# ddkang/avrecode

Hardware: AMD Instinct MI355X
Metric: input H.264 MB/s (compress+roundtrip) at 1/2/4/8 GPUs; bit-exact pass (higher is better)
Workload: dtype u8; 1 GPU; synthetic batch of independent 1080p CABAC I-slices (BASELINE configs[2]); slices_per_gpu=1024, model=parallel (the reference model reset per slice, SURVEY.md 7), input_bytes_per_gpu=261361164, recoded_bytes_C=258817967, bins=2511192484

## Files before the change

avrecode_amd/csrc/avr_walker.h:

```cpp
#pragma once
#include <type_traits>

#include "avr_slice_lds.h"

#define AVR_MB_LIKELY(x) (MODE == MODE_DECOMPRESS ? AVR_LIKELY(x) : (x))
#define AVR_MB_UNLIKELY(x) (MODE == MODE_DECOMPRESS ? AVR_UNLIKELY(x) : (x))

namespace avr {


template <int MODE, bool RM, bool FLD = false, bool P32 = false, bool SPL = false, bool SRD = false>
struct Walker {
  static constexpr bool DEC = MODE == MODE_COMPRESS || MODE == MODE_TRACE;
  const HotTables* T;
  const EngineTables* G;
  const avr_slice_desc* d;
  Shared* sh;
  typedef typename std::conditional<FLD, EdgeRec, EdgeCore>::type ERec;
  ERec* ring;
  uint32_t* mring;
  bool mring_global;
  uint16_t* est_g;
  uint8_t* frames;
  int64_t cur_off, prev_off;
  bool gmode;
  uint32_t* gsink;
  uint32_t gcount;
  InStream in;
  OutStream out;
  CabacDecoder cd;
  CabacEncoder ce;
  RecodedEncoder re;
  static constexpr bool VD = MODE == MODE_DECOMPRESS && !P32 && !RM && !SRD;
  typename std::conditional<P32, PDecoder, typename std::conditional<VD, VDecoder, RecodedDecoder>::type>::type rd;
  uint64_t rng;
  int W, H, mb_x, mb_y, slice_type, is_b, cat_, t8mode;
  int fld, fld_pic, my, ystep;
  int top_pending;
  AVR_FI int mrow() const { return FLD ? my : mb_y; }
  int mbaff;
  uint32_t pst, ring_cols;
  int left_ok, top_ok, last_dqp_nz;
  uint32_t cf, lf, tf;
  static constexpr uint32_t CF_8X8 = 0x80;
  uint32_t edge_src;
  int err, finished;
  uint32_t bins;
  int target_mbs, mbs_done, last_mb;
  int nref0, nref1, d8x8inf, x264_build, first_mb;
  const SeamRec* seam;
  uint8_t* snap;
  uint32_t* snap_count;
  uint32_t snap_cap, snap_n, snap_last, snap_q, split_bits, rec_stride, piece_mbs;
  int cut;
  AVR_FI bool seam_place(uint32_t bitpos, uint32_t offset, uint32_t* ce) const {
    if (bitpos < 26) return false;
    const uint32_t m = (bitpos - 10) >> 3, sb = m > 12 ? m - 12 : 0, e = (bitpos + 7) >> 3, r = 8 * e - bitpos;
    const uint32_t sub = offset << r;
    uint32_t borrow = 0, low = 0, q = ~0u, cache = 0;
    for (uint32_t j = e; j-- > sb;) {
      const uint32_t t = e - 1 - j;
      const uint32_t sbyte = t < 4 ? (sub >> (8 * t)) & 0xff : 0u;
      const uint32_t f = j < in.limit ? (uint32_t)in.g[j] : 0u;
      const uint32_t v = f - sbyte - borrow;
      borrow = v >> 31;
      const uint32_t z = v & 0xff;
      if (j >= m) low |= z << (8 * t);
      else if (q == ~0u && z != 0xff) q = j, cache = z;
    }
    if (borrow || q == ~0u) return false;
    const uint32_t lowbits = bitpos - 8 * m;
    ce[0] = (low >> r) & ((1u << lowbits) - 1);
    ce[1] = cd.range;
    ce[2] = m - 1 - q;
    ce[3] = cache;
    ce[4] = lowbits - 18;
    ce[5] = q;
    return true;
  }
  AVR_FI void seam_cut(int addr) {
    const uint32_t pos = cd_bitpos(cd);
    if (pos - snap_last < split_bits || (uint64_t)pos + split_bits / 2 > 8ull * d->payload_size) return;
    snap_last = pos;
    if (snap_n >= snap_cap) return;
    uint32_t ce[6];
    if (!seam_place(pos, cd.low >> cd.k, ce) || (snap_n && ce[5] <= snap_q)) return;
    snap_q = ce[5];
    rc_writeback();
    mc_store();
    uint32_t* r32 = (uint32_t*)(snap + (size_t)snap_n * rec_stride);
    const uint32_t lane = __lane_id();
    if (lane < 16) {
      const uint32_t v = lane == 0 ? (uint32_t)addr : lane == 1 ? (uint32_t)last_dqp_nz : lane == 2 ? cd.low
                       : lane == 3 ? cd.range : lane == 4 ? (uint32_t)cd.k : lane == 5 ? cd.next
                       : lane == 6 ? ce[0] : lane == 7 ? ce[1] : lane == 8 ? ce[2] : lane == 9 ? ce[3]
                       : lane == 10 ? ce[4] : lane == 11 ? ce[5] : 0u;
      r32[lane] = v;
    }
    const uint32_t* st = (const uint32_t*)sh->state;
    for (uint32_t i = lane; i < 256; i += 64) r32[16 + i] = st[i];
    const uint32_t* e = (const uint32_t*)ring;
    for (uint32_t i = lane; i < (uint32_t)W * 10; i += 64) r32[16 + 256 + i] = i % 10 ? e[i] : e[i] & ~kEdgeMringNz;
    snap_n++;
    if constexpr (MODE == MODE_COMPRESS) {
      push(OP_FINISH | OP_RESTART);
      publish();
      while (ld_volatile(&sh->fifo_tail[0]) != ring0.head) {
        __builtin_amdgcn_s_sleep(1);
      }
      for (uint32_t i = lane; i < (uint32_t)W * kMringDwords; i += 64) mring[i] = 0;
      wave_sync();
    }
  }
  uint32_t prio_cell, prio_cur;
  AVR_FI void update_prio() {
    const uint32_t pos = MODE == MODE_DECOMPRESS ? rd.next : cd.next;
    const uint32_t size = d->payload_size;
    const uint32_t rem = pos < size ? size - pos : 0u;
    cu_post(prio_cell, rem);
    const uint32_t p = cu_rank_prio(prio_cell, rem);
    if (p != prio_cur) {
      prio_cur = p;
      set_prio(p);
      if (__lane_id() == 0) *(volatile __attribute__((address_space(3))) uint32_t*)&sh->prio = p;
    }
  }
  RingOutT<MODE == MODE_DECOMPRESS> ring0;
  static constexpr bool kStageLevels = true;
// ... 418 lines not shown
        int sy, ry;
        left_src(fld, afrm, bottom, y4, 16, &sy, &ry);
        t8rows |= (((sy ? lb : lt) & F_T8) ? 1u : 0u) << y4;
      }
      int s = 0, dw = 0;
      if (L >= 1 && L < 13) {
        const int p = ((int)L - 1) >> 2;
        int r;
        left_src(fld, afrm, bottom, ((int)L - 1) & 3, (cat_ == 1 && p) ? 8 : 16, &s, &r);
        dw = 1 + p * 4 + min(r, 3);
      } else if (L >= 13 && L < 29) {
        const int k = ((int)L - 13) & 7;
        int r;
        left_src(fld, afrm, bottom, k >> 1, 16, &s, &r);
        dw = 13 + (((int)L - 13) >> 3) * 8 + r * 2 + (k & 1);
      } else if (L == 29 || L == 30 || L == 31) {
        s = s0;
        dw = (int)L;
      } else if (L >= 32 && L < 45) {
        s = bottom;
        dw = (int)L;
      }
      uint32_t v = L < 45 ? ((const uint32_t*)&lp[s])[dw] : 0u;
      const uint32_t v2 = (L >= 29 && L < 32) ? ((const uint32_t*)&lp[s2])[L] : 0u;
      if (L == 0) {
        v = t8rows | cbp << 16;
      } else if (L >= 13 && L < 29) {
        if (fld != (uint32_t)(!afrm)) v = scale_mvd(v, fld);
      } else if (L == 29 || L == 30 || L == 31) {
        const uint32_t b1 = (v >> (8 * ((r0 >> 1) * 2 + 1))) & 0xff, b3 = (v2 >> (8 * ((r2 >> 1) * 2 + 1))) & 0xff;
        v = (L == 31 ? 0u : 0xff00ffu) | b1 << 8 | b3 << 24;
        if (L != 31 && fld != (uint32_t)(!afrm)) v = scale_ref(v, fld);
      }
      if (L < 45) ((uint32_t*)&sh->left)[L] = v;
    }
    const int above = (at & F_DEC) != 0;
    const int sel = !fld ? (bottom ? 1 : above ? 2 : 0) : above ? ((!bottom && (at & F_FLD)) ? 1 : 2) : 0;
    const int msel = bottom ? 1 : above ? 2 : 0;
    uint32_t v = 0;
    if (L < 10 && sel) v = ((const uint32_t*)&pair_edge(sel - 1)[mb_x])[L];
    else if (L >= 10 && L < 23 && msel) v = ((const uint32_t*)&pair_edge(msel - 1)[mb_x])[L];
    const uint32_t t0 = __builtin_amdgcn_readlane(v, 0);
    if (sel && ((t0 & F_FLD) ? 1u : 0u) != fld) {
      if (L >= 4 && L < 8) v = scale_mvd(v, fld);
      else if (L == 8) v = scale_ref(v, fld);
    }
    if (L < 23) ((uint32_t*)&ring[mb_x])[L] = v;
    tf = t0;
    top_ok = sel != 0;
    wave_sync();
  }
  AVR_FI void mbaff_layer_begin() {
    const int bottom = (pst & PST_BOT) != 0;
    uint32_t fld = pst & PST_FLD;
    if (!bottom) {
      fld = mbaff_field_flag(fld);
      pst = (pst & ~PST_FLD) | fld;
    }
    if (fld) cf |= F_FLD;
    mbaff_view(bottom, fld);
  }

  AVR_FI int mnnz_left(int idx) const {
    if (RM) return frames[cur_off + ((int64_t)mrow() * W + mb_x - 1) * 52 + idx];
    return left_ok ? sh->left.mnnz[idx] : 0;
  }
  AVR_FI int mnnz_top(int idx) const {
    if (RM) return (FLD && top_pending) ? 0 : frames[cur_off + ((int64_t)(mrow() - 1) * W + mb_x) * 52 + idx];
    if (FLD && fld_pic) return 0;
    if constexpr (FLD) {
      return (top_ok | mbaff) ? ring[mb_x].mnnz[idx] : 0;
    } else {
      if (!top_ok) return 0;
      const uint32_t at = (uint32_t)mb_x * (kMringDwords * 4) + mring_dword((uint32_t)idx >> 2) * 4 + ((uint32_t)idx & 3);
      if (mring_global) return (tf & kEdgeMringNz) ? ((const __attribute__((address_space(1))) uint8_t*)mring)[at] : 0;
      return ((const __attribute__((address_space(3))) uint8_t*)mring)[at];
    }
  }
  AVR_FI int mnnz_prev(int idx) const {
    if (RM) return prev_off < 0 ? 0 : frames[prev_off + ((int64_t)mrow() * W + mb_x) * 52 + idx];
    return 0;
  }

  AVR_FI int nz_bits(int cat, int n, int max, int is_dc, int c422, int count) {
    const int bits = max > 16 ? 6 : max > 4 ? 4 : 2;
    if (MODE == MODE_COMPRESS && RM && gmode && !gsink) {
      gcount += (uint32_t)bits;
      return count & ((1 << bits) - 1);
    }
    int has_left, has_above, lv = 0, av = 0;
    if (n >= 48) {
      has_left = mb_x > 0;
      has_above = mrow() > 0;
      if (has_left) lv = mnnz_left(n);
      if (has_above) av = mnnz_top(n);
    } else {
      uint8_t L = T->nb_left[n], U = T->nb_up[n];
      int li = L & 63, ui = U & 63;
      if (max >= 32) { li &= ~3; ui &= ~3; }
      has_left = !(L & 128) || mb_x > 0;
      has_above = !(U & 128) || mrow() > 0;
      if (has_left) lv = (L & 128) ? mnnz_left(li) : sh->cur.mnnz[li];
      if (has_above) av = (U & 128) ? mnnz_top(ui) : sh->cur.mnnz[ui];
    }
    const int pv = mnnz_prev(n);
    const int t = (((cf & CF_8X8) || max > 32) ? 1 : 0) + 2 * is_dc + c422 + 4 * cat;
    if (MODE == MODE_COMPRESS) {
      const int i = (int)__lane_id();
      const int cur_bit = 1 << (i & 7);
      const int so_far = count & (cur_bit - 1);
      const int lb = has_left ? (lv >= cur_bit) : 2;
      const int ab = av ? (av >= cur_bit) : 2;
      const int pb = pv >= cur_bit;
      const int idx = kSigEst + (((((cur_bit - 1 + so_far) * 2 + pb) * 3 + lb) * 3 + ab) * 57 + t);
      push_v(op_model((count >> (i & 7)) & 1, OPM_CACHE, idx), (uint32_t)bits);
      return count & ((1 << bits) - 1);
    }
    if (MODE == MODE_DECOMPRESS) {
      const uint32_t L = __lane_id();
      const int i = 31 - __clz((int)L + 1);
      const int cur_bit = 1 << i;
      const int lb = has_left ? (lv >= cur_bit) : 2;
      const int ab = av ? (av >= cur_bit) : 2;
      const int pb = pv >= cur_bit;
      const uint32_t idx_v = kSigEst + ((((L * 2 + pb) * 3 + lb) * 3 + ab) * 57 + t);
      uint32_t e_v = 0, slot_v = 0;
      const bool hit = est_probe4(sh, idx_v, &e_v, &slot_v);
      const uint64_t hit_m = __ballot(hit);
      int so_far = 0;
      for (int k = 0; k < bits; k++) {
        const uint32_t j = (1u << k) - 1 + (uint32_t)so_far;
        const uint32_t idx = __builtin_amdgcn_readlane(idx_v, j);
        uint32_t e, slot;
        if ((hit_m >> j) & 1) {
          e = __builtin_amdgcn_readlane(e_v, j);
          slot = __builtin_amdgcn_readlane(slot_v, j);
        } else {
          e = est_load(sh, est_g, idx, &slot);
        }
        const int b = rdec(e);
        est_store(sh, est_g, idx, slot, est_update(e, b, 0x60));
        so_far |= b << k;
      }
      return so_far;
    }
    int so_far = 0;
    for (int i = 0; i < bits; i++) {
      const int cur_bit = 1 << i;
      const int lb = has_left ? (lv >= cur_bit) : 2;
      const int ab = av ? (av >= cur_bit) : 2;
      const int pb = pv >= cur_bit;
      const int idx = kSigEst + (((((cur_bit - 1 + so_far) * 2 + pb) * 3 + lb) * 3 + ab) * 57 + t);
      int b;
      if (MODE == MODE_COMPRESS) {
        b = (count >> i) & 1;
        push(op_model(b, OPM_CACHE, idx));
      } else {
        uint32_t slot;
        const uint32_t e = est_load(sh, est_g, idx, &slot);
        b = rdec(e);
        est_store(sh, est_g, idx, slot, est_update(e, b, 0x60));
      }
      if (b) so_far |= cur_bit;
    }
    return so_far;
  }

  AVR_FI int sig_est_index(int cat, int max, int is_dc, int c422, int zz, int nnz_m, int obs) const {
    if (max == 64) return T->sig_est_base[cat] + (T->sig8x8[zz] * 64 + nnz_m) * 64 + obs;
    int zo = (is_dc && c422) ? (zz < 2 ? 0 : zz < 4 ? 1 : 2) : zz;
    return T->sig_est_base[cat] + (zo * 16 + nnz_m) * 16 + obs;
  }

  AVR_FI int sig_map(int cat, int n, int max, int is_dc, int c422) {
    const int numc8x8 = cat_ == 2 ? 2 : 1;
    const int sb = T->sig_base[cat], lb = T->last_base[cat], seb = (int)opaque_u32((uint32_t)T->sig_est_base[cat]);
    const int bits = max > 16 ? 6 : max > 4 ? 4 : 2;
    const int mask = (1 << bits) - 1;
    int cnt = 0;
    if (DEC) {
      uint64_t sigmask = 0;
      int pos, end = max - 2;
      PROF_BEGIN(t3);
      if (MODE == MODE_TRACE) trace_map_begin(cat, n, max, is_dc, c422);
      auto map_loop = [&](auto K) {
        constexpr int k = decltype(K)::value;
        for (pos = 0; pos < max - 1; pos++) {
          int sc, lc;
          if constexpr (k == 2) {
            sc = (int)__builtin_amdgcn_readlane(sig8_v, (uint32_t)pos);
            lc = (int)__builtin_amdgcn_readlane(last8_v, (uint32_t)pos);
          } else if constexpr (k == 1) {
            sc = lc = min(pos / numc8x8, 2);
          } else {
            sc = lc = pos;
          }
          if (rdecide(sc)) {
            sigmask |= 1ull << pos;
            cnt++;
            if (rdecide(16 + lc)) { end = pos; break; }
          }
        }
      };
      if (max == 64) map_loop(std::integral_constant<int, 2>());
      else if (cat == 3) map_loop(std::integral_constant<int, 1>());
      else map_loop(std::integral_constant<int, 0>());
      if (pos == max - 1) cnt++;
      if (MODE == MODE_TRACE) trace_map_end();
      PROF_END(3, t3);
      if (MODE == MODE_COMPRESS) {
        PROF_BEGIN(t4);
        nz_bits(cat, n, max, is_dc, c422, cnt);
        PROF_END(4, t4);
        PROF_BEGIN(t5);
        const int nnz_m = cnt & mask;
        const int zz = (int)__lane_id();
        const int b = (int)((sigmask >> zz) & 1);
        const int obs = (int)__builtin_amdgcn_mbcnt_hi((uint32_t)(sigmask >> 32), __builtin_amdgcn_mbcnt_lo((uint32_t)sigmask, 0u));
        const int idx = sig_est_index(cat, max, is_dc, c422, zz, nnz_m, obs);
        push_v(op_model(b, OPM_CACHE | OPM_THR50, idx), (uint32_t)end + 1);
        PROF_END(5, t5);
      }
    } else if (MODE == MODE_DECOMPRESS) {
      PROF_BEGIN(t4);
      const int nnz_m = nz_bits(cat, n, max, is_dc, c422, 0);
      PROF_END(4, t4);
      PROF_BEGIN(t3);
      int pos;
      const uint32_t sop = opaque_u32((uint32_t)sb << 3 | OPK_DECISION << 1 | 1u << OPC_SHIFT_D);
      const uint32_t lop = opaque_u32((uint32_t)lb << 3 | OPK_DECISION << 1 | 2u << OPC_SHIFT_D);
      auto map_loop = [&](auto K) {
        constexpr int k = decltype(K)::value;
        constexpr int stride = k == 2 ? 64 : 16;
        uint32_t mk = 0;
        constexpr bool defer = k == 0;
        uint32_t dslot_v = 0, de_v = 0;
        for (pos = 0; pos < max - 1; pos++) {
          int sc, lc, zo;
          if constexpr (k == 2) {
            const uint32_t v = __builtin_amdgcn_readlane(sig8_v, (uint32_t)pos);
            sc = FLD ? (int)(v & 0xff) : (int)v;
            zo = FLD ? (int)(v >> 8) : (int)v;
            lc = (int)__builtin_amdgcn_readlane(last8_v, (uint32_t)pos);
          } else if constexpr (k == 1) {
            sc = lc = min(pos / numc8x8, 2);
            zo = (is_dc && c422) ? (pos < 2 ? 0 : pos < 4 ? 1 : 2) : pos;
          } else {
            sc = lc = zo = pos;
          }
          const int idx = seb + (zo * stride + nnz_m) * stride + cnt;
          uint32_t slot;
          uint32_t e = est_load(sh, est_g, idx, &slot, defer);
          int b = rdec(e);
          const uint32_t ne = est_update(e, b, 0x50);
          if (defer && AVR_LIKELY(slot >> 31)) {
            dslot_v = wlane(dslot_v, (uint32_t)pos, slot);
            de_v = wlane(de_v, (uint32_t)pos, ne);
          } else {
            est_store(sh, est_g, idx, slot, ne);
          }
          bins++;
          if constexpr (FLD) push(sop + ((uint32_t)sc << 3) + (uint32_t)b);
          else mk |= (uint32_t)b << (pos & 15);
          if (b) {
            cnt++;
            int last = nnz_m == cnt;
            bins++;
            if constexpr (FLD) push(lop + ((uint32_t)lc << 3) + (uint32_t)last);
            if (last) break;
          }
          if constexpr (!FLD && k == 2) {
            if ((pos & 15) == 15) {
              push(op_map(cat, 16, 0, mk));
              mk = 0;
            }
          }
        }
        if constexpr (defer) {
          if (dslot_v >> 31) sh->etab[dslot_v & 0xffff] = (dslot_v & 0xffff0000u) | de_v;
          wave_sync();
        }
        if constexpr (!FLD) {
          const int ended = pos < max - 1;
          push(op_map(cat, (pos & 15) + ended, ended, mk));
        }
      };
      if (max == 64) map_loop(std::integral_constant<int, 2>());
      else if (cat == 3) map_loop(std::integral_constant<int, 1>());
      else map_loop(std::integral_constant<int, 0>());
      if (pos == max - 1) cnt++;
      PROF_END(3, t3);
    } else {
      int pos;
      for (pos = 0; pos < max - 1; pos++) {
        int sc, lc;
        if (max == 64) {
          sc = (int)__builtin_amdgcn_readlane(sig8_v, (uint32_t)pos);
          lc = (int)__builtin_amdgcn_readlane(last8_v, (uint32_t)pos);
        }
        else if (cat == 3) { sc = lc = min(pos / numc8x8, 2); }
        else sc = lc = pos;
        if (rbin(sc, sb + sc)) {
          cnt++;
          if (rbin(16 + lc, lb + lc)) break;
        }
      }
      if (pos == max - 1) cnt++;
    }
    return cnt;
  }

  AVR_FI void residual_block(int cat, int n, int max, int is_dc, int c422, int p, int pw, int x4, int y4) {
    if (AVR_MB_UNLIKELY(err)) return;
    MbRec& cur = sh->cur;
    int coded = 1;
    if (max != 64 || cat_ == 3) {
      int nza, nzb;
      if (is_dc) {
        int bit = cat == 3 ? (0x40 << (n - 49)) : (0x100 << (n - 48));
        nza = (nb_cbp_left() & bit) != 0;
        nzb = (nb_cbp_top() & bit) != 0;
      } else {
        nza = nnz_left(p, pw, x4, y4) > 0;
        nzb = nnz_top(p, x4, y4) > 0;
      }
      rc_select(cat);
      coded = rbin(42 + nza + 2 * nzb, T->cbf_base[cat] + nza + 2 * nzb);
    }
    int cnt = 0;
    if (coded) {
      rc_select(cat);
      cnt = sig_map(cat, n, max, is_dc, c422);
      const int ab = (int)opaque_u32((uint32_t)T->abs_base[cat]);
      int gt1 = 0, eq1 = 0;
      PROF_BEGIN(t6);
      if constexpr (MODE == MODE_DECOMPRESS && !FLD) {
        for (int i = cnt - 1; i >= 0 && !err; i--) {
          int absl;
          const int i0 = gt1 ? 0 : min(4, 1 + eq1);
          if (!rdec_lane(32 + i0)) {
            absl = 1;
          } else {
            const int i1 = 5 + min(4 - (cat == 3), gt1);
            absl = 2;
            while (absl < 15 && rdec_lane(32 + i1)) absl++;
          }
          if (absl < 15) {
            push(op_level(cat, absl, rdec_bypass()));
          } else {
            push(op_level(cat, 15, 0));
            int k = 0;
            while (bypass(SE_LEVEL_SUFFIX, k)) {
              if (++k > 30) { err = AVR_SLICE_BAD_LEVEL; break; }
            }
            while (k-- > 0) bypass(SE_LEVEL_SUFFIX, 100);
            bypass(SE_OTHER, 0);
          }
          if (absl == 1) eq1++;
          else gt1++;
        }
      } else if constexpr (MODE == MODE_COMPRESS && kStageLevels) {
        const bool st = !(RM && gmode);
        auto lpush = [&](uint32_t op) {
          if (st) ring0.stage(op);
          else push(op);
        };
        auto lbyp = [&]() {
          bins++;
          const int b = cd_bypass(cd, in);
          lpush(op_model(b, 0, 1024));
          return b;
        };
        for (int i = cnt - 1; i >= 0 && !err; i--) {
          int absl;
          const int i0 = gt1 ? 0 : min(4, 1 + eq1);
          int b = rdecide(32 + i0);
          lpush(op_model(b, 0, ab + i0));
          if (!b) {
            absl = 1;
          } else {
            const int i1 = 5 + min(4 - (cat == 3), gt1);
            absl = 2;
            while (absl < 15) {
              b = rdecide(32 + i1);
              lpush(op_model(b, 0, ab + i1));
              if (!b) break;
              absl++;
            }
            if (absl >= 15) {
              int k = 0;
              while (lbyp()) {
                if (++k > 30) { err = AVR_SLICE_BAD_LEVEL; break; }
              }
              while (k-- > 0) lbyp();
            }
          }
          lbyp();
          if (absl == 1) eq1++;
          else gt1++;
        }
        if (st) ring0.flush_stage();
      } else
      for (int i = cnt - 1; i >= 0 && !err; i--) {
        int absl;
        const int i0 = gt1 ? 0 : min(4, 1 + eq1);
        if (!rbin(32 + i0, ab + i0)) {
          absl = 1;
        } else {
          const int i1 = 5 + min(4 - (cat == 3), gt1);
          absl = 2;
          while (absl < 15 && rbin(32 + i1, ab + i1)) absl++;
          if (absl >= 15) {
            int k = 0;
            while (bypass(SE_LEVEL_SUFFIX, k)) {
              if (++k > 30) { err = AVR_SLICE_BAD_LEVEL; break; }
            }
            int v = 1;
            while (k-- > 0) v += v + bypass(SE_LEVEL_SUFFIX, 100);
            absl = 14 + v;
          }
        }
        bypass(SE_OTHER, 0);
        if (absl == 1) eq1++;
        else gt1++;
      }
      PROF_END(6, t6);
      cur.mnnz[n] = (uint8_t)cnt;
      if (max > 32) cf |= CF_8X8;
    }
    if (is_dc) {
      if (cnt) cf |= (uint32_t)(cat == 3 ? (0x40 << (n - 49)) : (0x100 << (n - 48))) << 16;
    } else if (max == 64) {
      cur.nnz[p][y4 * 4 + x4] = cur.nnz[p][y4 * 4 + x4 + 1] = (uint8_t)cnt;
      cur.nnz[p][y4 * 4 + 4 + x4] = cur.nnz[p][y4 * 4 + 4 + x4 + 1] = (uint8_t)cnt;
    } else {
      cur.nnz[p][y4 * 4 + x4] = (uint8_t)cnt;
    }
  }

  AVR_FI void blk_pos(int n, int* x4, int* y4) const {
    int s = c_scan8[n];
    int row = s >> 3;
    *x4 = (s & 7) - 4;
    *y4 = row <= 4 ? row - 1 : row <= 9 ? row - 6 : row - 11;
  }

  AVR_FI int push_block(int nb, int cat, int n, int max, int is_dc, int c422, int p, int pw, int x4, int y4) {
    sh->blk[nb] = (uint32_t)cat | (uint32_t)n << 4 | (uint32_t)max << 10 | (uint32_t)is_dc << 17 |
                  (uint32_t)c422 << 18 | (uint32_t)p << 19 | (uint32_t)pw << 21 | (uint32_t)x4 << 24 |
                  (uint32_t)y4 << 26;
    return nb + 1;
  }
  AVR_FI int list_luma(int nb, int p, int i16, int cbp) {
    const int cat_dc = p == 0 ? 0 : p == 1 ? 6 : 10;
    const int cat_ac = cat_dc + 1, cat_4 = cat_dc + 2, cat_8 = p == 0 ? 5 : p == 1 ? 9 : 13;
    int x4, y4;
    if (i16) {
      nb = push_block(nb, cat_dc, 48 + p, 16, 1, 0, p, 4, 0, 0);
      if (cbp & 15)
        for (int i = 0; i < 16; i++) {
          blk_pos(16 * p + i, &x4, &y4);
          nb = push_block(nb, cat_ac, 16 * p + i, 15, 0, 0, p, 4, x4, y4);
        }
      return nb;
    }
    for (int i8 = 0; i8 < 4; i8++) {
      if (!(cbp & (1 << i8))) continue;
      if (cf & F_T8) {
        blk_pos(16 * p + 4 * i8, &x4, &y4);
        nb = push_block(nb, cat_8, 16 * p + 4 * i8, 64, 0, 0, p, 4, x4, y4);
      } else {
        for (int i4 = 0; i4 < 4; i4++) {
          int n = 16 * p + 4 * i8 + i4;
          blk_pos(n, &x4, &y4);
          nb = push_block(nb, cat_4, n, 16, 0, 0, p, 4, x4, y4);
        }
      }
    }
    return nb;
  }

  AVR_FI void residual(int i16, int cbp) {
    int nb = list_luma(0, 0, i16, cbp);
    if (cat_ == 3) {
      nb = list_luma(nb, 1, i16, cbp);
      nb = list_luma(nb, 2, i16, cbp);
    } else if (cat_ == 1 || cat_ == 2) {
      const int c422 = cat_ == 2;
      if (cbp & 0x30)
        for (int c = 0; c < 2; c++) nb = push_block(nb, 3, 49 + c, c422 ? 8 : 4, 1, c422, 1 + c, 2, 0, 0);
      if (cbp & 0x20)
        for (int c = 0; c < 2; c++)
          for (int i8 = 0; i8 < (c422 ? 2 : 1); i8++)
            for (int i = 0; i < 4; i++) {
              int n = 16 + 16 * c + 8 * i8 + i, x4, y4;
              blk_pos(n, &x4, &y4);
              nb = push_block(nb, 4, n, 15, 0, 0, 1 + c, 2, x4, y4);
            }
    }
    PROF_BEGIN(t2);
    for (int j = 0; j < nb && AVR_MB_LIKELY(!err); j++) {
      const uint32_t b = sh->blk[j];
      residual_block(b & 15, (b >> 4) & 63, (b >> 10) & 127, (b >> 17) & 1, (b >> 18) & 1, (b >> 19) & 3,
                     (b >> 21) & 7, (b >> 24) & 3, (b >> 26) & 3);
    }
    PROF_END(2, t2);
  }

  AVR_FI int ref_gt0(int list, int x4, int y4, int use_left) const {
    uint8_t dir;
    int r;
    if (use_left) {
      if (x4 > 0) {
        int b8 = (y4 >> 1) * 2 + ((x4 - 1) >> 1);
        dir = sh->cur.direct8[b8]; r = sh->cur.ref[list][b8];
      } else {
        if (!left_ok) return 0;
        int b8 = (y4 >> 1) * 2 + 1;
        dir = sh->left.direct8[b8]; r = sh->left.ref[list][b8];
      }
    } else {
      if (y4 > 0) {
        int b8 = ((y4 - 1) >> 1) * 2 + (x4 >> 1);
        dir = sh->cur.direct8[b8]; r = sh->cur.ref[list][b8];
      } else {
        if (!top_ok) return 0;
        dir = ring[mb_x].direct8[x4 >> 1]; r = ring[mb_x].ref[list][x4 >> 1];
      }
    }
    if (is_b && dir) return 0;
    return r > 0;
  }
  AVR_FI int decode_ref(int list, int x4, int y4) {
    int ctx = ref_gt0(list, x4, y4, 1) + 2 * ref_gt0(list, x4, y4, 0);
    int ref = 0;
    avr_limit = (list ? nref1 : nref0) - 1;
    while (bin(SE_REF, ref, 54 + ctx)) {
      ref++;
      ctx = (ctx >> 2) + 4;
      if (ref >= 32) { err = AVR_SLICE_BAD_REF_IDX; return 0; }
    }
    return ref;
  }
  AVR_FI int mvd_nb(int list, int comp, int x4, int y4, int use_left) const {
    if (use_left) {
      if (x4 > 0) return sh->cur.mvd[list][y4 * 4 + x4 - 1][comp];
      return left_ok ? sh->left.mvd[list][y4 * 4 + 3][comp] : 0;
    }
    if (y4 > 0) return sh->cur.mvd[list][(y4 - 1) * 4 + x4][comp];
    return top_ok ? ring[mb_x].mvd[list][x4][comp] : 0;
  }
  AVR_FI int decode_mvd(int list, int comp, int x4, int y4) {
    const int base = comp ? 47 : 40;
    const int amvd = mvd_nb(list, comp, x4, y4, 1) + mvd_nb(list, comp, x4, y4, 0);
    const int inc = amvd < 3 ? 0 : amvd <= 32 ? 1 : 2;
    if constexpr (MODE == MODE_DECOMPRESS && !FLD) {
      if (!rdec_mc(base + inc)) {
        push(op_mvd(comp, inc, 0, 0));
        return 0;
      }
      int mvd = 1, ctx = base + 3;
      while (mvd < 9 && rdec_mc(ctx)) {
        if (mvd < 4) ctx++;
        mvd++;
      }
// ... 333 lines not shown
  const int cols = (FLD && d->structure == AVR_STRUCT_MBAFF && (int)w.ring_cols >= 3 * w.W + 7) ? 3 * w.W + 7 : w.W;
  if (seam) {
    const uint32_t* e32 = (const uint32_t*)(seam + 1);
    for (int i = lane; i < w.W * kEdgeBytes / 4; i += nt) ring32[i] = i % 10 ? e32[i] : e32[i] & ~kEdgeMringNz;
    if (!w.mring_global)
      for (int i = lane; i < w.W * kMringDwords; i += nt) w.mring[i] = 0;
  } else {
    for (int i = lane; i < cols * (int)sizeof(typename Walker<MODE, RM, FLD, P32, SPL, SRD>::ERec) / 4; i += nt) ring32[i] = 0;
  }
  if (lane < 2) {
    w.sh->fifo_head[lane] = 0;
    w.sh->fifo_tail[lane] = 0;
  }
  __syncthreads();
}

template <int MODE, bool RM, bool FLD, bool P32, bool SPL, bool SRD>
AVR_FI void walk_slice(Walker<MODE, RM, FLD, P32, SPL, SRD>& w) {
  const avr_slice_desc* d = w.d;
  w.W = d->mb_width;
  w.H = (FLD && w.fld_pic) ? d->mb_height >> 1 : d->mb_height;
  w.slice_type = d->slice_type;
  w.is_b = d->slice_type == 1;
  w.cat_ = d->chroma_array_type;
  w.t8mode = d->transform_8x8_mode;
  w.nref0 = d->num_ref_idx_l0;
  w.nref1 = d->num_ref_idx_l1;
  w.d8x8inf = d->direct_8x8_inference;
  w.x264_build = d->x264_build;
  w.first_mb = d->first_mb;
  w.last_dqp_nz = 0;
  if constexpr (SPL) {
    if (w.seam) w.last_dqp_nz = (int)w.seam->last_dqp_nz;
  }
  w.err = 0;
  w.finished = 0;
  w.bins = 0;
  w.mbs_done = 0;
  int addr = d->first_mb;
  const int lane = threadIdx.x;
  const int npic = w.W * w.H;
  w.mb_x = addr % w.W;
  w.mb_y = addr / w.W;
  w.ystep = (FLD && w.fld_pic) ? 2 : 1;
  w.my = w.mb_y * w.ystep + (d->structure == AVR_STRUCT_BOTTOM_FIELD ? 1 : 0);
  w.mbaff = FLD && d->structure == AVR_STRUCT_MBAFF;
  w.pst = 0;
  if ((FLD && w.mbaff)) {
    if ((int)w.ring_cols < 3 * w.W + 7 || (addr & 1)) { w.err = AVR_SLICE_MBAFF_RING; return; }
    w.mb_x = (addr >> 1) % w.W;
    w.mb_y = (addr >> 1) / w.W;
    w.ystep = 2;
    w.my = 2 * w.mb_y;
  }
  {
    const int j = lane, ph_c = (w.cat_ == 2 || w.cat_ == 3) ? 4 : 2;
    int src = 0;
    if (j >= 1 && j < 4) src = 1 + (j - 1) * 4 + (j == 1 ? 3 : ph_c - 1);
    else if (j >= 4 && j < 8) src = 13 + ((j - 4) >> 1) * 8 + 6 + ((j - 4) & 1);
    else if (j == 8) src = 29;
    else if (j == 9) src = 31;
    else if (j >= 10 && j < 23) src = 32 + (j - 10);
    w.edge_src = (uint32_t)src;
  }
  for (;;) {
    if (AVR_MB_UNLIKELY(addr >= npic)) { w.err = AVR_SLICE_BAD_MB_ADDR; break; }
    if constexpr (SPL && MODE == MODE_COMPRESS) {
      if (AVR_MB_UNLIKELY(w.snap && w.mb_x == 0 && w.mbs_done > 0)) w.seam_cut(addr);
    }
    PROF_BEGINW(ps0);
    if (!(FLD && w.mbaff)) {
      w.left_ok = w.mb_x > 0 && addr - 1 >= w.first_mb;
      w.tf = *(const uint32_t*)&w.ring[w.mb_x];
      w.top_ok = (w.tf & F_DEC) != 0;
    } else if (!(w.pst & Walker<MODE, RM, FLD, P32, SPL, SRD>::PST_BOT)) {
      w.mbaff_pair_start();
    }
    w.cf = 0;
    {
      uint32_t* c32 = (uint32_t*)&w.sh->cur;
      if (lane < (int)sizeof(MbRec) / 4) c32[lane] = (lane == 29 || lane == 30) ? 0xffffffffu : 0u;
      wave_sync();
    }
    SPROF_ENDW(0, ps0);
#ifdef AVR_PROFILE
    w.sprofb[0]++;
#endif
    PROF_BEGINW(t1);
    w.decode_mb();
    PROF_ENDW(1, t1);
    PROF_BEGINW(t7);
    if (AVR_MB_UNLIKELY(w.err)) break;
    w.cf |= F_DEC;
    w.mbs_done++;
    w.last_mb = addr + 1 >= npic;
    wave_sync();
    {
      const uint32_t* c32 = (const uint32_t*)&w.sh->cur;
      const uint32_t v = c32[lane < 45 ? lane : 44];
      const uint32_t ve = c32[w.edge_src], ref1 = c32[30];
      const uint32_t ev = lane == 8 ? (ve >> 16) | (ref1 & 0xffff0000u) : lane == 9 ? ve >> 16 : ve;
      if (!(FLD && w.mbaff)) {
        uint32_t* l32 = (uint32_t*)&w.sh->left;
        if (lane < 45) l32[lane] = v;
        uint32_t* e32 = (uint32_t*)&w.ring[w.mb_x];
        if constexpr (FLD) {
          if (lane < 23) e32[lane] = lane == 0 ? (w.cf & 0xffff017fu) : ev;
        } else {
          const bool mz = !RM && w.mring_global &&
                          __ballot(lane >= 10 && lane < 23 && ((kMringUsed >> (lane - 10)) & 1) && ev != 0) != 0;
          if (lane < 10) e32[lane] = lane == 0 ? ((w.cf & 0xffff017fu) | (mz ? kEdgeMringNz : 0u)) : ev;
          else if (!RM && lane < 23 && ((kMringUsed >> (lane - 10)) & 1)) {
            const uint32_t at = (uint32_t)w.mb_x * kMringDwords + mring_dword((uint32_t)lane - 10);
            if (w.mring_global) {
              if (mz) ((__attribute__((address_space(1))) uint32_t*)w.mring)[at] = ev;
            } else {
              ((__attribute__((address_space(3))) uint32_t*)w.mring)[at] = ev;
            }
          }
        }
        w.lf = w.cf;
      } else {
        const int bot = (w.pst & Walker<MODE, RM, FLD, P32, SPL, SRD>::PST_BOT) != 0;
        uint32_t* e32 = (uint32_t*)&w.pair_edge(bot)[w.mb_x];
        if (lane < 23) e32[lane] = lane == 0 ? (w.cf & 0xffff017fu) : ev;
        uint32_t* pr = (uint32_t*)w.pair_rec();
        const uint32_t t = pr[lane < 45 ? lane : 44];
        if (!bot) {
          if (lane < 45) pr[lane] = lane == 0 ? w.cf : v;
        } else if (lane < 45) {
          pr[45 + lane] = t;
          pr[90 + lane] = lane == 0 ? w.cf : v;
        }
      }
      if (RM) {
        uint32_t* f32 = (uint32_t*)(w.frames + w.cur_off + ((int64_t)w.mrow() * w.W + w.mb_x) * 52);
        if (lane >= 32 && lane < 45) f32[lane - 32] = v;
      }
      wave_sync();
    }
    PROF_ENDW(7, t7);
    PROF_BEGINW(ps7);
    if (MODE == MODE_COMPRESS || MODE == MODE_DECOMPRESS) {
      w.publish();
      if (!RM) w.update_prio();
    }
    const int eos = (!(FLD && w.mbaff) || (w.pst & Walker<MODE, RM, FLD, P32, SPL, SRD>::PST_BOT)) ? w.terminate(SE_EOS) : 0;
    SPROF_ENDW(7, ps7);
    if (AVR_MB_UNLIKELY(eos)) break;
    if constexpr (SPL) {
      if (AVR_MB_UNLIKELY(w.piece_mbs && (uint32_t)w.mbs_done >= w.piece_mbs)) {
        w.finished = 1;
        w.cut = 1;
        break;
      }
    }
    if (Walker<MODE, RM, FLD, P32, SPL, SRD>::DEC && AVR_MB_UNLIKELY(w.in.limit && w.cd.next > w.in.limit + 8)) { w.err = AVR_SLICE_OVERREAD; break; }
    if (MODE == MODE_DECOMPRESS && !RM && AVR_MB_UNLIKELY(w.in.limit && w.rd.next > w.in.limit + 16)) { w.err = AVR_SLICE_OVERREAD; break; }
    addr++;
    if ((FLD && w.mbaff) && !(w.pst & Walker<MODE, RM, FLD, P32, SPL, SRD>::PST_BOT)) {
      w.pst |= Walker<MODE, RM, FLD, P32, SPL, SRD>::PST_BOT;
      w.my++;
      continue;
    }
    if ((FLD && w.mbaff)) {
      w.pst = 0;
      w.my--;
    }
    if (++w.mb_x == w.W) {
      w.mb_x = 0;
      w.mb_y++;
      if (FLD) w.my += w.ystep;
    }
  }
}

template <int MODE, bool RM, bool FLD, bool P32, bool SPL, bool SRD>
AVR_FI void begin_slice(Walker<MODE, RM, FLD, P32, SPL, SRD>& w, const avr_slice_desc* d, const uint8_t* in, uint8_t* out) {
  w.d = d;
  w.in.g = in + d->payload_offset;
  w.in.limit = MODE == MODE_GENERATE ? 0 : d->read_limit;
  w.in.lds = w.sh->in_stage;
  w.in.win = 0xffffffffu - kStage;
  w.out.g = out + d->out_offset;
  w.out.cap = d->out_capacity;
  w.out.n = 0;
  w.out.last = 0;
  w.ring0.init(w.sh, 0);
  vtab_load(w.vt, w.T);
  w.rc_cat = -1;
  w.rc_v = 0;
  w.fld_pic = FLD && (d->structure == AVR_STRUCT_TOP_FIELD || d->structure == AVR_STRUCT_BOTTOM_FIELD);
  w.fld = -1;
  if (FLD) w.set_fld(w.fld_pic);
  else w.sig8_v = w.T->sig8x8[__lane_id()];
  w.top_pending = 0;
  w.last8_v = w.T->last8x8[__lane_id()];
  if (MODE == MODE_DECOMPRESS) w.byp_e = w.sh->est[1024];
  w.mc_load();
  if (!RM && (MODE == MODE_COMPRESS || MODE == MODE_DECOMPRESS)) {
    if (w.prio_cell == kNoCell) w.prio_cell = cu_cell();
    w.prio_cur = 0xffffffffu;
  }
  if (MODE == MODE_COMPRESS || MODE == MODE_TRACE) {
    cd_init(w.cd, w.in);
    if constexpr (SPL) {
      if (w.seam) {
        w.cd.low = w.seam->cd_low;
        w.cd.range = w.seam->cd_range;
        w.cd.k = (int)w.seam->cd_k;
        w.cd.next = w.seam->cd_next;
      }
    }
  } else if (MODE == MODE_DECOMPRESS) {
    rd_init(w.rd, w.in);
  } else {
    ce_init(w.ce);
    w.rng = d->payload_offset * 0x9E3779B97F4A7C15ull + 0x1234567ull + (uint64_t)d->picture_id;
    w.target_mbs = d->payload_size ? (int)d->payload_size : 1 << 30;
  }
#ifdef AVR_PROFILE
  for (int i = 0; i < 8; i++) w.prof[i] = 0, w.profb[i] = 0, w.sprof[i] = 0, w.sprofb[i] = 0;
#endif
}

template <int MODE, bool RM, bool FLD, bool P32, bool SPL, bool SRD>
AVR_FI void profile_slice(Walker<MODE, RM, FLD, P32, SPL, SRD>& w) {
#ifdef AVR_PROFILE
  w.bins = 0;
  const uint64_t t0 = PROF_T();
  const uint32_t t0_b = 0;
  walk_slice(w);
  PROF_ENDW(0, t0);
  if (__lane_id() == 0) {
    for (int i = 0; i < 8; i++) {
      atomicAdd(&avr_prof[i], (unsigned long long)w.prof[i]);
      atomicAdd(&avr_prof[8 + i], (unsigned long long)w.profb[i]);
      atomicAdd(&avr_prof[32 + i], (unsigned long long)w.sprof[i]);
      atomicAdd(&avr_prof[40 + i], (unsigned long long)w.sprofb[i]);
    }
  }
#else
  walk_slice(w);
#endif
}

template <int MODE, bool RM, bool FLD, bool P32, bool SPL, bool SRD>
AVR_FI void walker_slice(Walker<MODE, RM, FLD, P32, SPL, SRD>& w, const avr_slice_desc* d, const uint8_t* in, avr_slice_result* res) {
  begin_slice(w, d, in, nullptr);
  profile_slice(w);
  if constexpr (SPL) {
    if (MODE == MODE_COMPRESS && w.snap && __lane_id() == 0) *w.snap_count = w.snap_n;
  }
  if (!RM) cu_post(w.prio_cell, 0);
  w.rc_writeback();
  w.mc_store();
  if (MODE == MODE_DECOMPRESS && __lane_id() == 0) w.sh->est[1024] = (uint16_t)w.byp_e;
  w.push(OP_END);
#ifdef AVR_PROFILE
  if (__lane_id() == 0) atomicAdd(&avr_prof[16], (unsigned long long)w.ring0.wait_cycles);
#endif
  w.publish();
  int status = w.err;
  if (!status && !w.finished) status = AVR_SLICE_NO_END;
  bool cut = false;
  if constexpr (SPL) {
    cut = w.cut;
    if (!status && w.piece_mbs && !cut) status = AVR_SLICE_NO_END;
  }
  int stop_ok = 1;
  if (MODE == MODE_COMPRESS && !status && !cut) {
    const uint32_t sbi = cd_bitpos(w.cd) - 1;
    const uint32_t k = sbi >> 3, size = d->payload_size;
    const uint32_t b = in_byte(w.in, k);
    const uint32_t masked = b & (0xffu << (7 - (sbi & 7))) & 0xff;
    if (masked == 0x80) stop_ok = (k == size) || (k + 1 == size);
    else stop_ok = (k + 1 == size) || (k + 2 == size && b == masked);
  }
  if (__lane_id() == 0) {
    w.sh->p_status = status;
// ... 11 lines not shown
```

Baseline: 172.4 MB/s.

## Keep per-MB residual block list and nnz neighbor state in wave registers

Builds the residual block list in parallel across lanes (one block per lane) and iterates it with readlane, instead of the serial list_luma path. Per-block nnz and model-nnz counts for the current MB, along with the left and top edge neighbors, are held in VGPRs and read with readlane. They are written back to LDS only once at the end of the MB, which replaces scattered LDS and global byte loads during context derivation. The cost is extra VGPR pressure, a per-MB edge preload, and more complex index packing that must stay bit-exact.

```diff
diff --git a/avrecode_amd/csrc/avr_walker.h b/avrecode_amd/csrc/avr_walker.h
--- a/avrecode_amd/csrc/avr_walker.h
+++ b/avrecode_amd/csrc/avr_walker.h
@@ -5,6 +5,10 @@
 
 #define AVR_MB_LIKELY(x) (MODE == MODE_DECOMPRESS ? AVR_LIKELY(x) : (x))
 #define AVR_MB_UNLIKELY(x) (MODE == MODE_DECOMPRESS ? AVR_UNLIKELY(x) : (x))
+
+#ifndef AVR_BLOCK_STATE
+#define AVR_BLOCK_STATE 3
+#endif
 
 namespace avr {
 
@@ -44,6 +48,11 @@
   uint32_t cf, lf, tf;
   static constexpr uint32_t CF_8X8 = 0x80;
   uint32_t edge_src;
+
+  static constexpr int BS = (!RM && !FLD && !SPL && !SRD) ? AVR_BLOCK_STATE : 0;
+  uint32_t blk_v, blk2_v;
+  uint32_t nz_v, nzn_v;
+  uint32_t mz_v, mzl_v, mzt_v;
   int err, finished;
   uint32_t bins;
   int target_mbs, mbs_done, last_mb;
@@ -628,13 +637,29 @@
     return 0;
   }
 
-  AVR_FI int nz_bits(int cat, int n, int max, int is_dc, int c422, int count) {
+  AVR_FI int nz_bits(int cat, int n, int max, int is_dc, int c422, int count, uint32_t b2 = 0) {
     const int bits = max > 16 ? 6 : max > 4 ? 4 : 2;
     if (MODE == MODE_COMPRESS && RM && gmode && !gsink) {
       gcount += (uint32_t)bits;
       return count & ((1 << bits) - 1);
     }
     int has_left, has_above, lv = 0, av = 0;
+    if constexpr (BS >= 3) {
+      if (n >= 48) {
+        has_left = mb_x > 0;
+        lv = (int)__builtin_amdgcn_readlane(mzl_v, (uint32_t)n);
+        av = (int)__builtin_amdgcn_readlane(mzt_v, (uint32_t)n);
+      } else {
+        const uint32_t L = (b2 >> 16) & 0xff, U = b2 >> 24;
+        uint32_t li = L & 63, ui = U & 63;
+        if (max >= 32) { li &= ~3u; ui &= ~3u; }
+        has_left = !(L & 128) || mb_x > 0;
+        const uint32_t lc = __builtin_amdgcn_readlane(mz_v, li), ln = __builtin_amdgcn_readlane(mzl_v, li);
+        const uint32_t uc = __builtin_amdgcn_readlane(mz_v, ui), un = __builtin_amdgcn_readlane(mzt_v, ui);
+        lv = (int)((L & 128) ? ln : lc);
+        av = (int)((U & 128) ? un : uc);
+      }
+    } else
     if (n >= 48) {
       has_left = mb_x > 0;
       has_above = mrow() > 0;
@@ -712,13 +737,13 @@
     return so_far;
   }
 
-  AVR_FI int sig_est_index(int cat, int max, int is_dc, int c422, int zz, int nnz_m, int obs) const {
-    if (max == 64) return T->sig_est_base[cat] + (T->sig8x8[zz] * 64 + nnz_m) * 64 + obs;
+  AVR_FI int sig_est_index(int seb, int max, int is_dc, int c422, int zz, int nnz_m, int obs) const {
+    if (max == 64) return seb + (T->sig8x8[zz] * 64 + nnz_m) * 64 + obs;
     int zo = (is_dc && c422) ? (zz < 2 ? 0 : zz < 4 ? 1 : 2) : zz;
-    return T->sig_est_base[cat] + (zo * 16 + nnz_m) * 16 + obs;
-  }
-
-  AVR_FI int sig_map(int cat, int n, int max, int is_dc, int c422) {
+    return seb + (zo * 16 + nnz_m) * 16 + obs;
+  }
+
+  AVR_FI int sig_map(int cat, int n, int max, int is_dc, int c422, uint32_t b2 = 0) {
     const int numc8x8 = cat_ == 2 ? 2 : 1;
     const int sb = T->sig_base[cat], lb = T->last_base[cat], seb = (int)opaque_u32((uint32_t)T->sig_est_base[cat]);
     const int bits = max > 16 ? 6 : max > 4 ? 4 : 2;
@@ -756,20 +781,20 @@
       PROF_END(3, t3);
       if (MODE == MODE_COMPRESS) {
         PROF_BEGIN(t4);
-        nz_bits(cat, n, max, is_dc, c422, cnt);
+        nz_bits(cat, n, max, is_dc, c422, cnt, b2);
         PROF_END(4, t4);
         PROF_BEGIN(t5);
         const int nnz_m = cnt & mask;
         const int zz = (int)__lane_id();
         const int b = (int)((sigmask >> zz) & 1);
         const int obs = (int)__builtin_amdgcn_mbcnt_hi((uint32_t)(sigmask >> 32), __builtin_amdgcn_mbcnt_lo((uint32_t)sigmask, 0u));
-        const int idx = sig_est_index(cat, max, is_dc, c422, zz, nnz_m, obs);
+        const int idx = sig_est_index(seb, max, is_dc, c422, zz, nnz_m, obs);
         push_v(op_model(b, OPM_CACHE | OPM_THR50, idx), (uint32_t)end + 1);
         PROF_END(5, t5);
       }
     } else if (MODE == MODE_DECOMPRESS) {
       PROF_BEGIN(t4);
-      const int nnz_m = nz_bits(cat, n, max, is_dc, c422, 0);
+      const int nnz_m = nz_bits(cat, n, max, is_dc, c422, 0, b2);
       PROF_END(4, t4);
       PROF_BEGIN(t3);
       int pos;
@@ -856,7 +881,7 @@
     return cnt;
   }
 
-  AVR_FI void residual_block(int cat, int n, int max, int is_dc, int c422, int p, int pw, int x4, int y4) {
+  AVR_FI void residual_block(int cat, int n, int max, int is_dc, int c422, int p, int pw, int x4, int y4, uint32_t b2 = 0) {
     if (AVR_MB_UNLIKELY(err)) return;
     MbRec& cur = sh->cur;
     int coded = 1;
@@ -866,6 +891,12 @@
         int bit = cat == 3 ? (0x40 << (n - 49)) : (0x100 << (n - 48));
         nza = (nb_cbp_left() & bit) != 0;
         nzb = (nb_cbp_top() & bit) != 0;
+      } else if constexpr (BS >= 2) {
+        const uint32_t ll = b2 & 63, tl = (b2 >> 8) & 63;
+        const uint32_t lc = __builtin_amdgcn_readlane(nz_v, ll), ln = __builtin_amdgcn_readlane(nzn_v, ll);
+        const uint32_t tc = __builtin_amdgcn_readlane(nz_v, tl), tn = __builtin_amdgcn_readlane(nzn_v, tl);
+        nza = ((b2 & 0x40) ? ln : lc) > 0;
+        nzb = ((b2 & 0x4000) ? tn : tc) > 0;
       } else {
         nza = nnz_left(p, pw, x4, y4) > 0;
         nzb = nnz_top(p, x4, y4) > 0;
@@ -876,7 +907,7 @@
     int cnt = 0;
     if (coded) {
       rc_select(cat);
-      cnt = sig_map(cat, n, max, is_dc, c422);
+      cnt = sig_map(cat, n, max, is_dc, c422, b2);
       const int ab = (int)opaque_u32((uint32_t)T->abs_base[cat]);
       int gt1 = 0, eq1 = 0;
       PROF_BEGIN(t6);
@@ -971,11 +1002,22 @@
         else gt1++;
       }
       PROF_END(6, t6);
-      cur.mnnz[n] = (uint8_t)cnt;
+      if constexpr (BS >= 3) mz_v = wlane(mz_v, (uint32_t)n, (uint32_t)cnt);
+      else cur.mnnz[n] = (uint8_t)cnt;
       if (max > 32) cf |= CF_8X8;
     }
     if (is_dc) {
       if (cnt) cf |= (uint32_t)(cat == 3 ? (0x40 << (n - 49)) : (0x100 << (n - 48))) << 16;
+    } else if constexpr (BS >= 2) {
+      if (cnt) {
+        const uint32_t g = (uint32_t)(p * 16 + y4 * 4 + x4);
+        nz_v = wlane(nz_v, g, (uint32_t)cnt);
+        if (max == 64) {
+          nz_v = wlane(nz_v, g + 1, (uint32_t)cnt);
+          nz_v = wlane(nz_v, g + 4, (uint32_t)cnt);
+          nz_v = wlane(nz_v, g + 5, (uint32_t)cnt);
+        }
+      }
     } else if (max == 64) {
       cur.nnz[p][y4 * 4 + x4] = cur.nnz[p][y4 * 4 + x4 + 1] = (uint8_t)cnt;
       cur.nnz[p][y4 * 4 + 4 + x4] = cur.nnz[p][y4 * 4 + 4 + x4 + 1] = (uint8_t)cnt;
@@ -1026,7 +1068,109 @@
     return nb;
   }
 
+  AVR_FI int list_build(int i16, int cbp) {
+    const int j = (int)__lane_id();
+    const int t8 = (cf & F_T8) != 0, m4 = cbp & 15;
+    const int np = i16 ? (m4 ? 17 : 1) : __builtin_popcount((uint32_t)m4) << (t8 ? 0 : 2);
+    const int nluma = cat_ == 3 ? 3 * np : np;
+    const int c422 = cat_ == 2, chroma = cat_ == 1 || cat_ == 2;
+    const int ndc = (chroma && (cbp & 0x30)) ? 2 : 0, per = c422 ? 8 : 4;
+    const int nac = (chroma && (cbp & 0x20)) ? 2 * per : 0;
+    const int p = (j >= np) + (j >= 2 * np), k = j - p * np;
+    const int cat_dc = p == 0 ? 0 : p == 1 ? 6 : 10;
+    int cat, i, max, is_dc = 0;
+    if (i16) {
+      is_dc = k == 0;
+      i = is_dc ? 0 : k - 1;
+      cat = cat_dc + !is_dc;
+      max = is_dc ? 16 : 15;
+    } else {
+      const int q = t8 ? k : k >> 2;
+      int i8 = 0;
+      for (int b = 1; b < 4; b++)
+        if (((m4 >> b) & 1) && __builtin_popcount((uint32_t)(m4 & ((1 << b) - 1))) == q) i8 = b;
+      i = 4 * i8 + (t8 ? 0 : (k & 3));
+      cat = t8 ? (p == 0 ? 5 : p == 1 ? 9 : 13) : cat_dc + 2;
+      max = t8 ? 64 : 16;
+    }
+    int n = is_dc ? 48 + p : 16 * p + i, pl = p, pw = 4, dc422 = 0;
+    if (j >= nluma) {
+      const int jc = j - nluma;
+      if (jc < ndc) {
+        cat = 3; n = 49 + jc; max = per; is_dc = 1; dc422 = c422; pl = 1 + jc; i = 0;
+      } else {
+        const int ja = jc - ndc, c = ja >= per, jp = ja - c * per;
+        i = (jp & 3) + 8 * (jp >> 2);
+        cat = 4; n = 16 + 16 * c + i; max = 15; is_dc = 0; pl = 1 + c;
+      }
+      pw = 2;
+    }
+    const int x4 = (i & 1) | ((i >> 1) & 2), y4 = ((i >> 1) & 1) | ((i >> 2) & 2);
+    blk_v = (uint32_t)cat | (uint32_t)n << 4 | (uint32_t)max << 10 | (uint32_t)is_dc << 17 | (uint32_t)dc422 << 18 |
+            (uint32_t)x4 << 19 | (uint32_t)y4 << 21 | (uint32_t)pl << 23 | (uint32_t)pw << 25;
+    if constexpr (BS >= 2) {
+      const int g = pl * 16 + y4 * 4 + x4;
+      const uint32_t l = x4 > 0 ? (uint32_t)(g - 1) : 0x40u | (uint32_t)(pl * 8 + y4);
+      const uint32_t u = y4 > 0 ? (uint32_t)(g - 4) : 0x40u | (uint32_t)(pl * 8 + 4 + x4);
+      uint32_t v = l | u << 8;
+      if constexpr (BS >= 3) {
+        const int nt = n < 48 ? n : 0;
+        const uint32_t tb = (uint32_t)T->nb_left[nt] << 16 | (uint32_t)T->nb_up[nt] << 24;
+        v |= n < 48 ? tb : 0u;
+      }
+      blk2_v = v;
+    }
+    return nluma + ndc + nac;
+  }
+
+  AVR_FI void edge_load() {
+    const uint32_t L = __lane_id();
+    {
+      const uint32_t pl = (L >> 3) < 3 ? L >> 3 : 2, r = L & 7;
+      const int dflt = (cf & F_INTRA) ? 64 : 0;
+      const int pwp = (pl && (cat_ == 1 || cat_ == 2)) ? 2 : 4;
+      int ov_l = 0, ov_t = 0;
+      const int has_ov_l = nnz_override(lf, &ov_l), has_ov_t = nnz_override(tf, &ov_t);
+      const int lval = sh->left.nnz[pl][(r & 3) * 4 + pwp - 1], tval = ring[mb_x].nnz[pl][r & 3];
+      const int lres = !left_ok ? dflt : has_ov_l ? ov_l : lval;
+      const int tres = !top_ok ? dflt : has_ov_t ? ov_t : tval;
+      nzn_v = (uint32_t)(r < 4 ? lres : tres);
+    }
+    if constexpr (BS >= 3) {
+      const uint32_t idx = L < 52 ? L : 51;
+      const uint32_t lval = sh->left.mnnz[idx];
+      mzl_v = (left_ok && L < 52) ? lval : 0u;
+      const bool kept = L < 52 && ((kMringUsed >> (L >> 2)) & 1);
+      const uint32_t at = (uint32_t)mb_x * (kMringDwords * 4) + mring_dword(idx >> 2) * 4 + (idx & 3);
+      uint32_t tval = 0;
+      if (kept && top_ok) {
+        if (mring_global) {
+          if (tf & kEdgeMringNz) tval = ((const __attribute__((address_space(1))) uint8_t*)mring)[at];
+        } else {
+          tval = ((const __attribute__((address_space(3))) uint8_t*)mring)[at];
+        }
+      }
+      mzt_v = tval;
+    }
+  }
+
   AVR_FI void residual(int i16, int cbp) {
+    if constexpr (BS >= 1) {
+      const int nb = list_build(i16, cbp);
+      if constexpr (BS >= 2) edge_load();
+      PROF_BEGIN(t2);
+      for (int j = 0; j < nb && AVR_MB_LIKELY(!err); j++) {
+        const uint32_t b = __builtin_amdgcn_readlane(blk_v, (uint32_t)j);
+        const uint32_t b2 = BS >= 2 ? __builtin_amdgcn_readlane(blk2_v, (uint32_t)j) : 0u;
+        if constexpr (BS >= 2)
+          residual_block(b & 15, (b >> 4) & 63, (b >> 10) & 127, (b >> 17) & 1, (b >> 18) & 1, 0, 0, (b >> 19) & 63, 0, b2);
+        else
+          residual_block(b & 15, (b >> 4) & 63, (b >> 10) & 127, (b >> 17) & 1, (b >> 18) & 1, (b >> 23) & 3,
+                         (b >> 25) & 7, (b >> 19) & 3, (b >> 21) & 3);
+      }
+      PROF_END(2, t2);
+      return;
+    }
     int nb = list_luma(0, 0, i16, cbp);
     if (cat_ == 3) {
       nb = list_luma(nb, 1, i16, cbp);
@@ -1526,6 +1670,8 @@
       if (lane < (int)sizeof(MbRec) / 4) c32[lane] = (lane == 29 || lane == 30) ? 0xffffffffu : 0u;
       wave_sync();
     }
+    if constexpr (Walker<MODE, RM, FLD, P32, SPL, SRD>::BS >= 2) w.nz_v = 0;
+    if constexpr (Walker<MODE, RM, FLD, P32, SPL, SRD>::BS >= 3) w.mz_v = 0;
     SPROF_ENDW(0, ps0);
 #ifdef AVR_PROFILE
     w.sprofb[0]++;
@@ -1538,6 +1684,12 @@
     w.cf |= F_DEC;
     w.mbs_done++;
     w.last_mb = addr + 1 >= npic;
+    if constexpr (Walker<MODE, RM, FLD, P32, SPL, SRD>::BS >= 2) {
+      if (lane < 48) ((uint8_t*)w.sh->cur.nnz)[lane] = (uint8_t)w.nz_v;
+    }
+    if constexpr (Walker<MODE, RM, FLD, P32, SPL, SRD>::BS >= 3) {
+      if (lane < 52) w.sh->cur.mnnz[lane] = (uint8_t)w.mz_v;
+    }
     wave_sync();
     {
       const uint32_t* c32 = (const uint32_t*)&w.sh->cur;
@@ -1640,6 +1792,7 @@
   else w.sig8_v = w.T->sig8x8[__lane_id()];
   w.top_pending = 0;
   w.last8_v = w.T->last8x8[__lane_id()];
+  w.blk_v = w.blk2_v = w.nz_v = w.nzn_v = w.mz_v = w.mzl_v = w.mzt_v = 0;
   if (MODE == MODE_DECOMPRESS) w.byp_e = w.sh->est[1024];
   w.mc_load();
   if (!RM && (MODE == MODE_COMPRESS || MODE == MODE_DECOMPRESS)) {
```

Result: faster. 174.7 MB/s (median of 6 runs) (+1.3%).
